# wq2012/SpectralCluster

Measured on AMD Instinct MI355X. Metric: predict() calls/sec, n=8192 d=256 ICASSP2018 (GraphCut, eigengap k in [2,20], cosine k-means), higher is better.
Workload: dtype f64; 1 GPU; icassp2018_graphcut_n8192_d256_k8_max20; n_samples=8192, n_features=256, parallelism=replicas x1, collectives=none

## Files before the change

### spectralcluster_amd/csrc/diffuse_free.hip

```cpp
#include <algorithm>
#include <cstring>
#include <mutex>

#include "dpp.h"
#include "sc_internal.h"

namespace sc {

typedef int v4i __attribute__((ext_vector_type(4)));
typedef int v16i __attribute__((ext_vector_type(16)));

namespace {

__device__ __forceinline__ double fr_wave_max(double v) {
#pragma unroll
  for (int o = 32; o > 0; o >>= 1) v = fmax(v, __shfl_xor(v, o));
  return v;
}
__device__ __forceinline__ double fr_wave_sum(double v) {
#pragma unroll
  for (int o = 32; o > 0; o >>= 1) v += __shfl_xor(v, o);
  return v;
}
__device__ __forceinline__ double fr_block_max(double v, double* sm) {
// ... 574 lines not shown
__global__ __launch_bounds__(kI8Threads) void k_gemm_i8_sym_g(const GroupOf<I8GroupItem> g) {
  const I8GroupItem& a = g.s[blockIdx.y];
  const int nt = (a.n + kI8Tile - 1) / kI8Tile;
  if (a.n <= 0 || (int)blockIdx.x >= nt * (nt + 1) / 2) return;
  const int Kp = (a.n + 63) / 64 * 64;
  I8Split sp{0, 1, nullptr};
  sp.plan = a.plan;
  sp.cus = 0;
  sp.total = a.total;
  gemm_i8_sym_body<0>(a.Q, (size_t)2 * Kp, Kp / 64, a.tilemap, 0, a.T32, nt, a.n, a.M, nullptr, sp);
}

__global__ __launch_bounds__(kI8Threads) void k_i8_tail_finish(
    const int* __restrict__ wsp, int parts, int full_tiles, const int2* __restrict__ tilemap,
    float* __restrict__ T32, int nt, int n, unsigned* __restrict__ M,
    const int* __restrict__ plan, int cus, int nstages, const int* __restrict__ total) {
  const int tt = blockIdx.x, cq = blockIdx.y, cb = cq >> 2, q = cq & 3;
  int I, J;
  if (plan != nullptr) {
    __shared__ int pref[512];
    const int count = *total;
    int r;
    i8_split_plan(count, cus, nstages, &r, &parts);
    if (parts < 2 || tt >= r) return;
    plan_scan(plan, nt, pref);
    __syncthreads();
    full_tiles = count - r;
    plan_lookup(plan, nt, pref, full_tiles + tt, &I, &J);
  } else {
    const int2 tij = tilemap[full_tiles + tt];
    I = tij.x;
    J = tij.y;
  }
  const int lane = threadIdx.x & 63, w = threadIdx.x >> 6;
  const int rr = lane & 31, g = lane >> 5, wr = w >> 1, wc = w & 1;
  const int4* ws = reinterpret_cast<const int4*>(wsp) + (size_t)tt * parts * 24 * kI8Threads + threadIdx.x;
  int4 a = make_int4(0, 0, 0, 0), b = a, c = a;
  for (int p = 0; p < parts; ++p) {
    const int4* src = ws + (size_t)p * 24 * kI8Threads;
    const int4 x = src[(size_t)cq * kI8Threads];
    const int4 y = src[(size_t)(8 + cq) * kI8Threads];
    const int4 z = src[(size_t)(16 + cq) * kI8Threads];
    a.x += x.x; a.y += x.y; a.z += x.z; a.w += x.w;
    b.x += y.x; b.y += y.y; b.z += y.z; b.w += y.w;
    c.x += z.x; c.y += z.y; c.z += z.z; c.w += z.w;
  }
  const int hh[4] = {a.x, a.y, a.z, a.w}, mid[4] = {b.x, b.y, b.z, b.w}, ll[4] = {c.x, c.y, c.z, c.w};
  float* out = T32 + (size_t)tile_to_slot(I, J, nt) * (kI8Tile * kI8Tile);
  const int col = 64 * wc + 32 * cb + rr;
  const bool col_ok = J * kI8Tile + col < n;
  float colm = -INFINITY;
#pragma unroll
  for (int e = 0; e < 4; ++e) {
    const int row = 32 * wr + e + 8 * q + 4 * g;
    const double t = (double)hh[e] * 65536.0 + (double)mid[e] * 256.0 + (double)ll[e];
    const float tf = (float)t;
    out[row * kI8Tile + col] = tf;
    if (I * kI8Tile + row < n) colm = fmaxf(colm, tf);
    float v = col_ok ? tf : -INFINITY;
#pragma unroll
    for (int o = 16; o > 0; o >>= 1) v = fmaxf(v, __shfl_xor(v, o));
    if (rr == 0 && I * kI8Tile + row < n && v > -INFINITY)
      atomicMax(&M[I * kI8Tile + row], ordered_bits(v));
  }
  colm = fmaxf(colm, __shfl_xor(colm, 32));
  if (g == 0 && I != J && J * kI8Tile + col < n && colm > -INFINITY)
    atomicMax(&M[J * kI8Tile + col], ordered_bits(colm));
}

__device__ __forceinline__ void free_append(int row, int col, int cap, int* __restrict__ count,
                                            int* __restrict__ cand) {
  const int pos = atomicAdd(&count[row], 1);
  if (pos < cap) cand[(size_t)row * cap + pos] = col;
}

__device__ __forceinline__ void t32_candidates_body(
    const float* __restrict__ T32, int nt, int n, const unsigned* __restrict__ M,
    const double* __restrict__ R, const unsigned long long* __restrict__ rmax_bits, int cap,
    int* __restrict__ count, int* __restrict__ cand, const int* __restrict__ plan) {
  __shared__ float thrI[128], thrJ[128];
  int I, J;
  size_t slot = blockIdx.x;
  if (plan != nullptr) {
    __shared__ int pref[512];
    const int tiles_run = count[n + kPlanTotalWord];
    if (blockIdx.x == 0 && threadIdx.x == 0) count[n + 67] = tiles_run;
    if ((int)blockIdx.x >= tiles_run) return;
    plan_scan(plan, nt, pref);
    __syncthreads();
    plan_lookup(plan, nt, pref, blockIdx.x, &I, &J);
    slot = tile_to_slot(I, J, nt);
  } else {
    slot_to_tile(blockIdx.x, nt, &I, &J);
    if (blockIdx.x == 0 && threadIdx.x == 0) count[n + 67] = nt * (nt + 1) / 2;
  }
  const float* tile = T32 + slot * (kI8Tile * kI8Tile);
  const int r0 = I * kI8Tile, c0 = J * kI8Tile;
  const int c4 = 4 * (threadIdx.x & 31);
  float4 tv[16];
#pragma unroll
  for (int rg = 0; rg < 16; ++rg)
    tv[rg] = *reinterpret_cast<const float4*>(tile + (8 * rg + (threadIdx.x >> 5)) * kI8Tile + c4);
  const double Rmax = __longlong_as_double((long long)*rmax_bits);
  if (blockIdx.x == 0 && threadIdx.x == 0 && rmax_bits[1] != 0ull) atomicMax(count + n, 1 << 20);
  if (threadIdx.x < 128) {
    const int row = r0 + threadIdx.x;
    thrI[threadIdx.x] = row < n ? free_threshold(ordered_value(M[row]), R[row], Rmax, n) : INFINITY;
  } else {
    const int row = c0 + threadIdx.x - 128;
    thrJ[threadIdx.x - 128] =
        (row < n && I != J) ? free_threshold(ordered_value(M[row]), R[row], Rmax, n) : INFINITY;
  }
  __syncthreads();
  const float tj0 = thrJ[c4], tj1 = thrJ[c4 + 1], tj2 = thrJ[c4 + 2], tj3 = thrJ[c4 + 3];
  const float tjmin = fminf(fminf(tj0, tj1), fminf(tj2, tj3));
#pragma unroll
  for (int rg = 0; rg < 16; ++rg) {
    const int r = 8 * rg + (threadIdx.x >> 5);
    const float4 v = tv[rg];
    const float ti = thrI[r];
    const float vmax = fmaxf(fmaxf(v.x, v.y), fmaxf(v.z, v.w));
    if (vmax >= ti) {
      const int c = c0 + c4;
      if (v.x >= ti && c < n) free_append(r0 + r, c, cap, count, cand);
      if (v.y >= ti && c + 1 < n) free_append(r0 + r, c + 1, cap, count, cand);
      if (v.z >= ti && c + 2 < n) free_append(r0 + r, c + 2, cap, count, cand);
      if (v.w >= ti && c + 3 < n) free_append(r0 + r, c + 3, cap, count, cand);
    }
    if (vmax >= tjmin && r0 + r < n) {
      if (v.x >= tj0) free_append(c0 + c4, r0 + r, cap, count, cand);
      if (v.y >= tj1) free_append(c0 + c4 + 1, r0 + r, cap, count, cand);
      if (v.z >= tj2) free_append(c0 + c4 + 2, r0 + r, cap, count, cand);
      if (v.w >= tj3) free_append(c0 + c4 + 3, r0 + r, cap, count, cand);
    }
  }
}
__global__ __launch_bounds__(256) void k_t32_candidates(
    const float* __restrict__ T32, int nt, int n, const unsigned* __restrict__ M,
    const double* __restrict__ R, const unsigned long long* __restrict__ rmax_bits, int cap,
    int* __restrict__ count, int* __restrict__ cand, const int* __restrict__ plan) {
  t32_candidates_body(T32, nt, n, M, R, rmax_bits, cap, count, cand, plan);
}
__global__ __launch_bounds__(256) void k_t32_candidates_g(const GroupOf<FreeItem> g, int cap) {
  const FreeItem& a = g.s[blockIdx.y];
  const int nt = (a.n + kI8Tile - 1) / kI8Tile;
  if (a.n <= 0 || (int)blockIdx.x >= nt * (nt + 1) / 2) return;
  t32_candidates_body(a.T32, nt, a.n, reinterpret_cast<const unsigned*>(a.words), a.R,
                      reinterpret_cast<const unsigned long long*>(a.scal) + 2, cap, a.words + a.n,
                      a.cand, a.plan);
}


constexpr int kFreeCapMax = 8;
template <int CNT, int U>
__device__ __forceinline__ void free_row_dots(const double* __restrict__ x,
                                               const double* const* __restrict__ xj,
                                               const bool* self, const double* __restrict__ y1,
                                               int n, double* rs_out, double* acc_out) {
  double rs = 0.0;
  double acc[CNT > 0 ? CNT : 1];
#pragma unroll
  for (int c = 0; c < CNT; ++c) acc[c] = 0.0;
  for (int k0 = 2 * threadIdx.x; k0 < n; k0 += 512 * U) {
    double2 a[U], yy[U], b[U][CNT > 0 ? CNT : 1];
#pragma unroll
    for (int u = 0; u < U; ++u) {
      const int k = k0 + 512 * u;
      const bool in = k < n;
      a[u] = in ? *reinterpret_cast<const double2*>(x + k) : make_double2(0.0, 0.0);
      yy[u] = in ? *reinterpret_cast<const double2*>(y1 + k) : make_double2(0.0, 0.0);
#pragma unroll
      for (int c = 0; c < CNT; ++c)
        b[u][c] = (in && !self[c]) ? *reinterpret_cast<const double2*>(xj[c] + k)
                                   : make_double2(0.0, 0.0);
    }
#pragma unroll
    for (int u = 0; u < U; ++u) {
      const int k = k0 + 512 * u;
      if (k + 1 >= n) {
        a[u].y = 0.0;
        yy[u].y = 0.0;
#pragma unroll
        for (int c = 0; c < CNT; ++c) b[u][c].y = 0.0;
      }
      rs = __builtin_fma(a[u].x, yy[u].x, rs);
      rs = __builtin_fma(a[u].y, yy[u].y, rs);
#pragma unroll
      for (int c = 0; c < CNT; ++c) {
        const double2 bb = self[c] ? a[u] : b[u][c];
        acc[c] = __builtin_fma(a[u].x, bb.x, acc[c]);
        acc[c] = __builtin_fma(a[u].y, bb.y, acc[c]);
      }
    }
  }
  *rs_out = rs;
#pragma unroll
  for (int c = 0; c < CNT; ++c) acc_out[c] = acc[c];
}

__device__ __forceinline__ void free_row_stats_body(
    const double* __restrict__ A, int n, int ld, const double* __restrict__ y1,
    const int* __restrict__ count, const int* __restrict__ cand, int cap,
    double* __restrict__ rowmax, double* __restrict__ rowsum, int* __restrict__ ovf) {
  __shared__ double sm[4];
  const int row = blockIdx.x;
  const int total = count[row];
  const int cnt = total < cap ? total : cap;
  const double* x = A + (size_t)row * ld;
  const double* xj[kFreeCapMax];
  bool self[kFreeCapMax];
#pragma unroll
  for (int c = 0; c < kFreeCapMax; ++c) {
    const int j = c < cnt ? cand[(size_t)row * cap + c] : row;
    self[c] = j == row;
    xj[c] = A + (size_t)j * ld;
  }
  double acc[kFreeCapMax];
#pragma unroll
  for (int c = 0; c < kFreeCapMax; ++c) acc[c] = 0.0;
  double rs = 0.0;
  switch (cnt) {
    case 0: free_row_dots<0, 4>(x, xj, self, y1, n, &rs, acc); break;
    case 1: free_row_dots<1, 4>(x, xj, self, y1, n, &rs, acc); break;
    case 2: free_row_dots<2, 4>(x, xj, self, y1, n, &rs, acc); break;
    case 3: free_row_dots<3, 2>(x, xj, self, y1, n, &rs, acc); break;
    case 4: free_row_dots<4, 2>(x, xj, self, y1, n, &rs, acc); break;
    default: free_row_dots<kFreeCapMax, 1>(x, xj, self, y1, n, &rs, acc); break;
  }
  rs = fr_block_sum(rs, sm);
  double best = -INFINITY;
#pragma unroll
  for (int c = 0; c < kFreeCapMax; ++c) {
    if (c < cnt) {
      const double d = fr_block_sum(acc[c], sm);
      best = fmax(best, d);
    }
  }
  if (threadIdx.x == 0) {
    rowmax[row] = best;
    rowsum[row] = rs;
    if (total > cap) {
      const int e = atomicAdd(&ovf[0], 1);
      if (e < 64) ovf[1 + e] = row;
    }
  }
  if (row == 0) {
    int sum = 0, big = 0;
    for (int i = threadIdx.x; i < n; i += 256) {
      const int t = count[i];
      sum += t < cap ? t : cap;
      big = t > big ? t : big;
    }
#pragma unroll
    for (int o = 32; o > 0; o >>= 1) {
      sum += __shfl_xor(sum, o);
      const int other = __shfl_xor(big, o);
      big = other > big ? other : big;
    }
    __shared__ int ssum[4], sbig[4];
    if ((threadIdx.x & 63) == 0) {
      ssum[threadIdx.x >> 6] = sum;
      sbig[threadIdx.x >> 6] = big;
    }
    __syncthreads();
    if (threadIdx.x == 0) {
      ovf[65] = (ssum[0] + ssum[1]) + (ssum[2] + ssum[3]);
      ovf[66] = max(max(sbig[0], sbig[1]), max(sbig[2], sbig[3]));
    }
  }
}
__global__ __launch_bounds__(256) void k_free_row_stats(
    const double* __restrict__ A, int n, int ld, const double* __restrict__ y1,
    const int* __restrict__ count, const int* __restrict__ cand, int cap,
    double* __restrict__ rowmax, double* __restrict__ rowsum, int* __restrict__ ovf) {
  free_row_stats_body(A, n, ld, y1, count, cand, cap, rowmax, rowsum, ovf);
}
__global__ __launch_bounds__(256) void k_free_row_stats_g(const GroupOf<FreeItem> g, int cap) {
  const FreeItem& a = g.s[blockIdx.y];
  if ((int)blockIdx.x >= a.n) return;
  free_row_stats_body(a.A, a.n, a.ld, a.y1, a.words + a.n, a.cand, cap, a.rowmax, a.rowsum,
                       a.words + 2 * (size_t)a.n);
}

__global__ __launch_bounds__(256) void k_free_gather_rows(const double* __restrict__ A, int n,
                                                          int ld, const int* __restrict__ rows,
                                                          int nrows, double* __restrict__ Vs) {
  const int v = threadIdx.x & (kEigBlock - 1);
  const int k = blockIdx.x * (256 / kEigBlock) + threadIdx.x / kEigBlock;
  if (k >= n) return;
  Vs[(size_t)k * kEigBlock + v] = v < nrows ? A[(size_t)rows[v] * ld + k] : 0.0;
}
__global__ __launch_bounds__(256) void k_free_colmax(const double* __restrict__ W, int n,
                                                     const int* __restrict__ rows, int nrows,
                                                     double* __restrict__ rowmax) {
  __shared__ double sm[4];
  const int v = blockIdx.x;
  if (v >= nrows) return;
  double m = -INFINITY;
  for (int k = threadIdx.x; k < n; k += 256) m = fmax(m, W[(size_t)k * kEigBlock + v]);
  m = fr_block_max(m, sm);
  if (threadIdx.x == 0) rowmax[rows[v]] = m;
}

int free_rows_padded(int n) { return round_up(n, kI8Tile); }
int free_k_padded(int n) { return round_up(n, 64); }
size_t free_q_bytes(int n) { return (size_t)free_rows_padded(n) * 2 * free_k_padded(n); }
size_t free_t32_bytes(int n) {
  const size_t nt = (n + kI8Tile - 1) / kI8Tile;
  return nt * (nt + 1) / 2 * kI8Tile * kI8Tile * sizeof(float);
}
int free_candidate_cap() { return kFreeCapMax; }

void launch_free_absmax(hipStream_t s, const double* A, int n, int ld, double* scal) {
  hipLaunchKernelGGL(k_free_absmax, dim3(n), dim3(256), 0, s, A, n, ld,
                     reinterpret_cast<unsigned long long*>(scal));
}

void launch_free_amax_from_cut(hipStream_t s, const double* cut, int n, double p,
                               double floor_value, double* scal) {
  hipLaunchKernelGGL(k_free_amax_from_cut, dim3(1), dim3(256), 0, s, cut, n, p, floor_value, scal);
}

void launch_free_quantize(hipStream_t s, const double* A, int n, int ld, signed char* Q,
                          double* scal, double* y1, double* R, double* q2part) {
  const int Kp = free_k_padded(n);
  SC_OPT_IN_LDS(k_free_quantize<0>, 2 * 65536);
  hipLaunchKernelGGL(k_free_quantize<0>, dim3(free_rows_padded(n)), dim3(256), (size_t)2 * Kp, s, A,
                     n, ld, Q, (size_t)2 * Kp, Kp, scal, y1, R,
                     reinterpret_cast<unsigned long long*>(scal) + 2, q2part);
}
size_t free_q2part_bytes(int n) { return (size_t)free_k_padded(n) * (free_k_padded(n) / 64) * sizeof(double); }
size_t free_mx64_bytes(int n) { return (size_t)(free_k_padded(n) / 64) * (free_k_padded(n) / 64) * sizeof(double); }
size_t free_tau64_bytes(int n) { return (size_t)(free_k_padded(n) / 64) * sizeof(float); }
size_t free_plan_bytes(int n) {
  const size_t nt = (n + kI8Tile - 1) / kI8Tile;
  return (nt + nt * nt) * sizeof(int);
}
void launch_free_seg_reduce(hipStream_t s, const double* R, int n, const FreeSegs& segs) {
  const int nblk = free_k_padded(n) / 64;
  hipLaunchKernelGGL(k_free_seg_reduce, dim3(nblk), dim3(256), 0, s, R, n, nblk, segs);
}
void launch_free_tile_flags(hipStream_t s, const double* mx64, const float* tau64, int n,
                            int* plan, bool prune, int* words) {
  const int nt = (n + kI8Tile - 1) / kI8Tile;
  hipLaunchKernelGGL(k_free_tile_flags, dim3(nt), dim3(kFlagThreads), 0, s, mx64, tau64, nt,
                     free_k_padded(n) / 64, plan, prune ? 1 : 0,
                     words + 2 * (size_t)n + kPlanTotalWord);
}

static int device_cus() {
  static int cus = 0;
  if (cus == 0) {
    int dev = 0, v = 0;
    if (hipGetDevice(&dev) == hipSuccess &&
        hipDeviceGetAttribute(&v, hipDeviceAttributeMultiprocessorCount, dev) == hipSuccess && v > 0)
      cus = v;
    else
      cus = 256;
  }
  return cus;
}
void free_i8_split_plan(int n, int* tail_tiles, int* parts) {
  const int nt = (n + kI8Tile - 1) / kI8Tile;
  const int tiles = nt * (nt + 1) / 2;
  const int stages = free_k_padded(n) / 64;
  const int cus = device_cus();
  *tail_tiles = 0;
  *parts = 1;
  const int r = tiles % cus;
  if (tiles <= cus || r == 0 || 2 * r > cus) return;
  for (int f = std::min(8, cus / r); f >= 2; --f)
    if (stages % f == 0 && stages / f >= 4) {
      *tail_tiles = r;
      *parts = f;
      return;
    }
}
size_t free_i8_split_bytes(int n) {
  int r, f;
  free_i8_split_plan(n, &r, &f);
  return f > 1 ? (size_t)r * f * 96 * kI8Threads * sizeof(int) : 0;
}
size_t free_i8_split_bytes_plan() { return (size_t)device_cus() * 96 * kI8Threads * sizeof(int); }

void launch_gemm_i8_sym(hipStream_t s, const signed char* Q, int n, const int2* tilemap,
                        float* T32, unsigned* M, int* split_ws, const int* plan) {
  const int nt = (n + kI8Tile - 1) / kI8Tile;
  const int tiles = nt * (nt + 1) / 2;
  const int Kp = free_k_padded(n);
  const int lds = kI8Buffers * kI8StageBytes;
  if (plan != nullptr && split_ws != nullptr) {
    const int cus = device_cus();
    I8Split sp{0, 1, split_ws};
    sp.plan = plan;
    sp.cus = cus;
    sp.total = reinterpret_cast<const int*>(M) + 2 * (size_t)n + kPlanTotalWord;
    SC_OPT_IN_LDS(k_gemm_i8_sym<0>, lds);
    hipLaunchKernelGGL(k_gemm_i8_sym<0>, dim3(tiles + cus), dim3(kI8Threads), lds, s, Q,
                       (size_t)2 * Kp, Kp / 64, tilemap, 0, T32, nt, n, M,
                       static_cast<unsigned long long*>(nullptr), sp);
    hipLaunchKernelGGL(k_i8_tail_finish, dim3(cus / 2, 8), dim3(kI8Threads), 0, s, split_ws, 1, 0,
                       tilemap, T32, nt, n, M, plan, cus, Kp / 64, sp.total);
    return;
  }
  int r = 0, f = 1;
  if (split_ws != nullptr) free_i8_split_plan(n, &r, &f);
  const int full = tiles - r;
  const int xcd_chunk = (full % 8 == 0 && full >= 512) ? full / 8 : 0;
  SC_OPT_IN_LDS(k_gemm_i8_sym<0>, lds);
  hipLaunchKernelGGL(k_gemm_i8_sym<0>, dim3(full + r * f), dim3(kI8Threads), lds, s, Q,
                     (size_t)2 * Kp, Kp / 64, tilemap, xcd_chunk, T32, nt, n, M,
                     static_cast<unsigned long long*>(nullptr), I8Split{full, f, split_ws});
  if (f > 1)
    hipLaunchKernelGGL(k_i8_tail_finish, dim3(r, 8), dim3(kI8Threads), 0, s, split_ws, f, full,
                       tilemap, T32, nt, n, M, static_cast<const int*>(nullptr), 0, 0,
                       static_cast<const int*>(nullptr));
}

void launch_gemm_i8_sym_group(hipStream_t s, const signed char* const* Q, float* const* T32,
                              unsigned* const* M, int count, const int* ns,
                              const int2* const* tilemaps, const int* const* plans) {
  const int lds = kI8Buffers * kI8StageBytes;
  SC_OPT_IN_LDS(k_gemm_i8_sym_g, lds);
  GroupOf<I8GroupItem> g;
  memset(&g, 0, sizeof(g));
  int tiles = 0;
  for (int z = 0; z < count; ++z) {
    g.s[z] = I8GroupItem{Q[z], T32[z], M[z], tilemaps[z], ns[z], plans ? plans[z] : nullptr,
                         reinterpret_cast<const int*>(M[z]) + 2 * (size_t)ns[z] + kPlanTotalWord};
    const int nt = (ns[z] + kI8Tile - 1) / kI8Tile;
    tiles = std::max(tiles, nt * (nt + 1) / 2);
  }
  if (tiles == 0) return;
  hipLaunchKernelGGL(k_gemm_i8_sym_g, dim3(tiles, count), dim3(kI8Threads), lds, s, g);
}

void launch_t32_candidates(hipStream_t s, const float* T32, int n, const unsigned* M,
                           const double* R, const double* scal, int* count, int* cand,
                           const int* plan) {
  const int nt = (n + kI8Tile - 1) / kI8Tile;
  hipLaunchKernelGGL(k_t32_candidates, dim3(nt * (nt + 1) / 2), dim3(256), 0, s, T32, nt, n, M, R,
                     reinterpret_cast<const unsigned long long*>(scal) + 2, kFreeCapMax, count,
                     cand, plan);
}

void launch_free_row_stats(hipStream_t s, const double* A, int n, int ld, const double* y1,
                           const int* count, const int* cand, double* rowmax, double* rowsum,
                           int* ovf) {
  hipLaunchKernelGGL(k_free_row_stats, dim3(n), dim3(256), 0, s, A, n, ld, y1, count, cand,
                     kFreeCapMax, rowmax, rowsum, ovf);
}

static GroupOf<FreeItem> free_pack(const FreeItem* items, int count, int* nmax) {
  GroupOf<FreeItem> g;
  memset(&g, 0, sizeof(g));
  *nmax = 0;
  for (int z = 0; z < count; ++z) {
    g.s[z] = items[z];
    *nmax = std::max(*nmax, items[z].n);
  }
  return g;
}
void launch_free_begin_group(hipStream_t s, const FreeItem* items, int count, double floor_value,
                             bool pad_rows) {
  int nmax;
  const GroupOf<FreeItem> g = free_pack(items, count, &nmax);
  if (nmax == 0) return;
  const int nwords = 2 * nmax + kFreeOvfWords;
  hipLaunchKernelGGL(k_free_begin_g, dim3(1 + (nwords + 1023) / 1024 + (pad_rows ? 32 : 0), count),
                     dim3(256), 0, s, g, floor_value, pad_rows ? 1 : 0);
}
void launch_free_tile_flags_group(hipStream_t s, const FreeItem* items, int count, bool prune) {
  int nmax;
  const GroupOf<FreeItem> g = free_pack(items, count, &nmax);
  if (nmax == 0) return;
  hipLaunchKernelGGL(k_free_tile_flags_g, dim3((nmax + kI8Tile - 1) / kI8Tile, count),
                     dim3(kFlagThreads), 0, s, g, prune ? 1 : 0);
}
void launch_free_scan_stats_group(hipStream_t s, const FreeItem* items, int count) {
  int nmax;
  const GroupOf<FreeItem> g = free_pack(items, count, &nmax);
  if (nmax == 0) return;
  const int nt = (nmax + kI8Tile - 1) / kI8Tile;
  hipLaunchKernelGGL(k_t32_candidates_g, dim3(nt * (nt + 1) / 2, count), dim3(256), 0, s, g,
                     kFreeCapMax);
  hipLaunchKernelGGL(k_free_row_stats_g, dim3(nmax, count), dim3(256), 0, s, g, kFreeCapMax);
}

void launch_free_gather_rows(hipStream_t s, const double* A, int n, int ld, const int* rows,
                             int nrows, double* Vs) {
  const int per = 256 / kEigBlock;
  hipLaunchKernelGGL(k_free_gather_rows, dim3((n + per - 1) / per), dim3(256), 0, s, A, n, ld,
                     rows, nrows, Vs);
}

void launch_free_colmax(hipStream_t s, const double* W, int n, const int* rows, int nrows,
                        double* rowmax) {
  hipLaunchKernelGGL(k_free_colmax, dim3(nrows), dim3(256), 0, s, W, n, rows, nrows, rowmax);
}

}
```

### spectralcluster_amd/csrc/eig.hip

```cpp
#include <algorithm>
#include <cstring>
#include <mutex>

#include "sc_internal.h"

namespace sc {

typedef double v4f64 __attribute__((ext_vector_type(4)));
constexpr int B = kEigBlock;
constexpr int RB = 256 / B;
static_assert(B == 8 || B == 16, "block width must divide the 16-wide MFMA tile");

__device__ __forceinline__ uint64_t splitmix64(uint64_t x) {
  x += 0x9E3779B97F4A7C15ull;
  x = (x ^ (x >> 30)) * 0xBF58476D1CE4E5B9ull;
  x = (x ^ (x >> 27)) * 0x94D049BB133111EBull;
  return x ^ (x >> 31);
}
__device__ __forceinline__ double hash_uniform(uint64_t seed, uint64_t idx) {
  const uint64_t h = splitmix64(seed ^ splitmix64(idx));
  return (double)(h >> 11) * (2.0 / 9007199254740992.0) - 1.0;
}

__global__ void k_random_block(double* W, int n, uint64_t seed) {
// ... 68 lines not shown
      if (row < n && li < B)
        W[(size_t)row * B + li] =
            __builtin_fma(cvec ? cvec[row] : 1.0, sum,
                          pvec ? pvec[row] * V[(size_t)row * ldv + li] : 0.0);
    }
  }
}
__global__ __launch_bounds__(64 * kMvWaves) void k_block_matvec(
    const double* __restrict__ S, int ld, int n, const double* __restrict__ cvec,
    const double* __restrict__ pvec, const double* __restrict__ V, int ldv,
    const double* __restrict__ Vs, double* __restrict__ W) {
  block_matvec_body(S, ld, n, cvec, pvec, V, ldv, Vs, W);
}
__global__ __launch_bounds__(64 * kMvWaves) void k_block_matvec_g(const GroupOf<MatvecItem> g) {
  const MatvecItem& a = g.s[blockIdx.y];
  if ((int)blockIdx.x * 16 >= a.n) return;
  block_matvec_body(a.S, a.ld, a.n, a.cvec, a.pvec, a.V, a.ldv, a.Vs, a.W);
}

constexpr int kSymTile = 128;
constexpr int kSymPitch = 34;
__device__ __forceinline__ int sym_item_id(int I, int J, int nt) {
  return I * nt - I * (I - 1) / 2 + (J - I);
}
__device__ __forceinline__ void block_matvec_sym_body(
    const double* __restrict__ S, int ld, int n, const double* __restrict__ Vs,
    double* __restrict__ pdirect, double* __restrict__ pmirror, int nt) {
  __shared__ __attribute__((aligned(16))) double smem[4 * 32 * kSymPitch];
  int I = 0, rem = blockIdx.x, rowlen = nt;
  while (rem >= rowlen) {
    rem -= rowlen;
    --rowlen;
    ++I;
  }
  const int J = I + rem;
  const bool diag = I == J;
  const int lane = threadIdx.x & 63, wave = threadIdx.x >> 6;
  const int li = lane & 15, lg = lane >> 4;
  const int r0 = I * kSymTile + 32 * wave;
  const int c0 = J * kSymTile;
  double* patch = smem + wave * (32 * kSymPitch);
  double bm[8];
#pragma unroll
  for (int t = 0; t < 8; ++t) {
    const int row = r0 + 4 * t + lg;
    bm[t] = (row < n && li < B) ? Vs[(size_t)row * B + li] : 0.0;
  }
  v4f64 accd[2] = {{0.0, 0.0, 0.0, 0.0}, {0.0, 0.0, 0.0, 0.0}};
  v4f64 accm[4][2];
#pragma unroll
  for (int cs = 0; cs < 4; ++cs)
#pragma unroll
    for (int ct = 0; ct < 2; ++ct) accm[cs][ct] = (v4f64){0.0, 0.0, 0.0, 0.0};
  double2 a[1][2][4];
  auto load = [&](int buf, int cs) {
#pragma unroll
    for (int rt = 0; rt < 2; ++rt) {
      int row = r0 + 16 * rt + li;
      row = row < n ? row : n - 1;
      const double* src = S + (size_t)row * ld + c0 + 32 * cs + 2 * lg;
#pragma unroll
      for (int q = 0; q < 4; ++q) {
        if (c0 + 32 * cs + 8 * q + 2 * lg + 1 < ld)
          a[buf][rt][q] = *reinterpret_cast<const double2*>(src + 8 * q);
        else
          a[buf][rt][q] = make_double2(0.0, 0.0);
      }
    }
  };
#pragma unroll
  for (int cs = 0; cs < 4; ++cs) {
    constexpr int cur = 0;
    load(cur, cs);
    const int kb = c0 + 32 * cs + 2 * lg;
#pragma unroll
    for (int rt = 0; rt < 2; ++rt) {
      const bool rok = r0 + 16 * rt + li < n;
#pragma unroll
      for (int q = 0; q < 4; ++q) {
        if (!rok || kb + 8 * q >= n) a[cur][rt][q].x = 0.0;
        if (!rok || kb + 8 * q + 1 >= n) a[cur][rt][q].y = 0.0;
      }
    }
    double b[8];
#pragma unroll
    for (int t = 0; t < 8; ++t) {
      const int k = kb + 8 * (t >> 1) + (t & 1);
      b[t] = (k < n && li < B) ? Vs[(size_t)k * B + li] : 0.0;
    }
#pragma unroll
    for (int rt = 0; rt < 2; ++rt)
#pragma unroll
      for (int q = 0; q < 4; ++q) {
        accd[rt] = __builtin_amdgcn_mfma_f64_16x16x4f64(a[cur][rt][q].x, b[2 * q], accd[rt], 0, 0, 0);
        accd[rt] = __builtin_amdgcn_mfma_f64_16x16x4f64(a[cur][rt][q].y, b[2 * q + 1], accd[rt], 0, 0, 0);
      }
    if (!diag) {
#pragma unroll
      for (int rt = 0; rt < 2; ++rt)
#pragma unroll
        for (int q = 0; q < 4; ++q)
          *reinterpret_cast<double2*>(patch + (16 * rt + li) * kSymPitch + 8 * q + 2 * lg) =
              a[cur][rt][q];
      __builtin_amdgcn_fence(__ATOMIC_RELEASE, "wavefront");
      __builtin_amdgcn_wave_barrier();
#pragma unroll
      for (int ct = 0; ct < 2; ++ct)
#pragma unroll
        for (int t = 0; t < 8; ++t) {
          const double at = patch[(4 * t + lg) * kSymPitch + 16 * ct + li];
          accm[cs][ct] = __builtin_amdgcn_mfma_f64_16x16x4f64(at, bm[t], accm[cs][ct], 0, 0, 0);
        }
      __builtin_amdgcn_fence(__ATOMIC_ACQUIRE, "wavefront");
      __builtin_amdgcn_wave_barrier();
    }
  }
  const size_t item = blockIdx.x;
  if (li < B) {
#pragma unroll
    for (int rt = 0; rt < 2; ++rt)
#pragma unroll
      for (int r = 0; r < 4; ++r)
        pdirect[(item * kSymTile + 32 * wave + 16 * rt + lg + 4 * r) * B + li] = accd[rt][r];
  }
  if (diag) return;
  __syncthreads();
  double* red = smem;
  if (li < B) {
#pragma unroll
    for (int cs = 0; cs < 4; ++cs)
#pragma unroll
      for (int ct = 0; ct < 2; ++ct)
#pragma unroll
        for (int r = 0; r < 4; ++r)
          red[(wave * kSymTile + 32 * cs + 16 * ct + lg + 4 * r) * B + li] = accm[cs][ct][r];
  }
  __syncthreads();
  for (int e = threadIdx.x; e < kSymTile * B; e += 256)
    pmirror[item * (kSymTile * B) + e] =
        ((red[e] + red[kSymTile * B + e]) + red[2 * kSymTile * B + e]) + red[3 * kSymTile * B + e];
}
__global__ __launch_bounds__(256) void k_block_matvec_sym(
    const double* __restrict__ S, int ld, int n, const double* __restrict__ Vs,
    double* __restrict__ pdirect, double* __restrict__ pmirror, int nt) {
  block_matvec_sym_body(S, ld, n, Vs, pdirect, pmirror, nt);
}
__global__ __launch_bounds__(256) void k_block_matvec_sym_g(const GroupOf<MatvecItem> g) {
  const MatvecItem& a = g.s[blockIdx.y];
  const int nt = (a.n + kSymTile - 1) / kSymTile;
  if ((int)blockIdx.x >= nt * (nt + 1) / 2) return;
  block_matvec_sym_body(a.S, a.ld, a.n, a.Vs, a.slabs, a.slabs + (size_t)(nt * (nt + 1) / 2) * kSymTile * B, nt);
}

__device__ __forceinline__ void matvec_sym_reduce_body(
    const double* __restrict__ pdirect, const double* __restrict__ pmirror, int nt, int n,
    const double* __restrict__ cvec, const double* __restrict__ pvec,
    const double* __restrict__ V, int ldv, double* __restrict__ W) {
  const int R = blockIdx.x / 4;
  const int e = (blockIdx.x & 3) * 256 + threadIdx.x;
  const int rl = e / B, v = e % B;
  const int row = R * kSymTile + rl;
  double acc = 0.0;
  const int total = nt;
  for (int s0 = 0; s0 < total; s0 += 8) {
    double x[8];
#pragma unroll
    for (int u = 0; u < 8; ++u) {
      const int sidx = s0 + u;
      x[u] = 0.0;
      if (sidx < nt - R) {
        x[u] = pdirect[(size_t)sym_item_id(R, R + sidx, nt) * (kSymTile * B) + e];
      } else if (sidx < total) {
        x[u] = pmirror[(size_t)sym_item_id(sidx - (nt - R), R, nt) * (kSymTile * B) + e];
      }
    }
#pragma unroll
    for (int u = 0; u < 8; ++u) acc += x[u];
  }
  if (row < n) W[(size_t)row * B + v] =
      __builtin_fma(cvec ? cvec[row] : 1.0, acc, pvec ? pvec[row] * V[(size_t)row * ldv + v] : 0.0);
}
__global__ __launch_bounds__(256) void k_matvec_sym_reduce(
    const double* __restrict__ pdirect, const double* __restrict__ pmirror, int nt, int n,
    const double* __restrict__ cvec, const double* __restrict__ pvec,
    const double* __restrict__ V, int ldv, double* __restrict__ W) {
  matvec_sym_reduce_body(pdirect, pmirror, nt, n, cvec, pvec, V, ldv, W);
}
__global__ __launch_bounds__(256) void k_matvec_sym_reduce_g(const GroupOf<MatvecItem> g) {
  const MatvecItem& a = g.s[blockIdx.y];
  const int nt = (a.n + kSymTile - 1) / kSymTile;
  if ((int)blockIdx.x >= nt * 4) return;
  matvec_sym_reduce_body(a.slabs, a.slabs + (size_t)(nt * (nt + 1) / 2) * kSymTile * B, nt, a.n,
                         a.cvec, a.pvec, a.V, a.ldv, a.W);
}

constexpr int kProjGroups = 256 / B;
constexpr int kProjAcc = (kLdq + kProjGroups - 1) / kProjGroups;
__global__ __launch_bounds__(256) void k_proj_partial(
    const double* __restrict__ Q, int ldq, int m, const double* __restrict__ W,
    int n, double* __restrict__ partial) {
  __shared__ double Ql[8][kLdq];
  __shared__ double Wl[8][B];
  const int tid = threadIdx.x;
  const int jj = tid % B, ig = tid / B;
  const int rows_per = (n + gridDim.x - 1) / gridDim.x;
  const int rbeg = blockIdx.x * rows_per;
  const int rend = min(n, rbeg + rows_per);
  double acc[kProjAcc];
#pragma unroll
  for (int q = 0; q < kProjAcc; ++q) acc[q] = 0.0;
  for (int r = rbeg; r < rend; r += 8) {
    __syncthreads();
    for (int e = tid; e < 8 * m; e += 256) {
      const int rr = e / m, i = e - rr * m;
      Ql[rr][i] = (r + rr < rend) ? Q[(size_t)(r + rr) * ldq + i] : 0.0;
    }
    if (tid < 8 * B) {
      const int rr = tid / B;
      Wl[rr][jj] = (r + rr < rend) ? W[(size_t)(r + rr) * B + jj] : 0.0;
    }
    __syncthreads();
#pragma unroll
    for (int rr = 0; rr < 8; ++rr) {
      const double w = Wl[rr][jj];
#pragma unroll
      for (int q = 0; q < kProjAcc; ++q)
        if (ig + kProjGroups * q < m)
          acc[q] = __builtin_fma(Ql[rr][ig + kProjGroups * q], w, acc[q]);
    }
  }
  double* out = partial + (size_t)blockIdx.x * (kLdq * B);
#pragma unroll
  for (int q = 0; q < kProjAcc; ++q)
    if (ig + kProjGroups * q < m) out[(ig + kProjGroups * q) * B + jj] = acc[q];
}

__global__ __launch_bounds__(256) void k_reduce_H(
    const double* __restrict__ partial, int nparts, int m, double* __restrict__ Hbuf,
    double* __restrict__ T, int ldt, int col0, int accumulate,
    double* __restrict__ hsq) {
  __shared__ double sq[32];
  const int tid = threadIdx.x;
  const int sub = tid & 7;
  const int e = blockIdx.x * 32 + (tid >> 3);
  double h = 0.0;
  if (e < m * B)
    for (int g = sub; g < nparts; g += 8) h += partial[(size_t)g * (kLdq * B) + e];
  h += __shfl_xor(h, 1);
  h += __shfl_xor(h, 2);
  h += __shfl_xor(h, 4);
  if (sub == 0) {
    if (e < m * B) {
      Hbuf[e] = h;
      if (T != nullptr) {
        const int i = e / B, j = col0 + (e % B);
        if (i <= j) {
          const double v = accumulate ? T[(size_t)i * ldt + j] + h : h;
          T[(size_t)i * ldt + j] = v;
          T[(size_t)j * ldt + i] = v;
        }
      }
    } else {
      h = 0.0;
    }
    sq[tid >> 3] = h * h;
  }
  __syncthreads();
  if (tid < B) {
    double s = 0.0;
    for (int q = tid; q < 32; q += B) s += sq[q];
    atomicAdd(&hsq[tid], s);
  }
}

__global__ __launch_bounds__(256) void k_update_block(
    const double* __restrict__ Q, int ldq, int m, const double* __restrict__ Hbuf,
    double* __restrict__ W, int n) {
  __shared__ double Hl[kLdq * B];
  __shared__ double Ql[RB][kLdq + 1];
  const int tid = threadIdx.x;
  const int jj = tid % B, rr = tid / B;
  const int r0 = blockIdx.x * RB;
  for (int e = tid; e < m * B; e += 256) Hl[e] = Hbuf[e];
  for (int e = tid; e < RB * m; e += 256) {
    const int a = e / m, i = e - a * m;
    Ql[a][i] = (r0 + a < n) ? Q[(size_t)(r0 + a) * ldq + i] : 0.0;
  }
  __syncthreads();
  const int r = r0 + rr;
  if (r < n) {
    double acc = W[(size_t)r * B + jj];
    for (int i = 0; i < m; ++i) acc = __builtin_fma(-Ql[rr][i], Hl[i * B + jj], acc);
    W[(size_t)r * B + jj] = acc;
  }
}

__device__ __forceinline__ void chol8_wave(const double* G, double* __restrict__ Rinv,
                                           const double* __restrict__ hsq,
                                           int* __restrict__ flags,
                                           int* __restrict__ defect_flag, int flag_mode,
                                           int* __restrict__ sticky_flag = nullptr,
                                           int sticky_m = 0, bool sticky_on_defect = true);

__global__ __launch_bounds__(256) void k_reduce_chol(
    const double* __restrict__ partial, int nparts, double* __restrict__ Rinv,
    double* __restrict__ Gsave, const double* __restrict__ hsq,
    int* __restrict__ flags, int* __restrict__ defect_flag, int flag_mode) {
  static_assert(B == 8, "the factorisation below maps the 8 x 8 matrix onto one wavefront");
  __shared__ double G[B * B];
  const int tid = threadIdx.x;
  {
    constexpr int kLanes = 256 / (B * B);
    const int e = tid / kLanes, sub = tid % kLanes;
    double g = 0.0;
    for (int q = sub; q < nparts; q += kLanes) g += partial[(size_t)q * (kLdq * B) + e];
#pragma unroll
    for (int o = 1; o < kLanes; o <<= 1) g += __shfl_xor(g, o);
    if (sub == 0) {
      G[e] = g;
      if (Gsave) Gsave[e] = g;
    }
  }
  __syncthreads();
  if (tid >= 64) return;
  chol8_wave(G, Rinv, hsq, flags, defect_flag, flag_mode);
}

__device__ __forceinline__ void chol8_wave(const double* G, double* __restrict__ Rinv,
                                           const double* __restrict__ hsq,
                                           int* __restrict__ flags,
// ... 965 lines not shown
```

Measured before the change: 385.9 calls/s.

## Process two rows per block in free row stats and widen sym-reduce batch

The free-row-stats kernel now handles two rows per block. When a candidate neighbour is the other row in the block, its data comes from the already-loaded row registers instead of a second global read, and the block reductions are merged into a single shared-memory pass with one barrier. The launch grids are halved to match. Separately, the symmetric matvec reduction loads 32 partial slabs per batch instead of 8 to expose more memory-level parallelism. The cost is higher register pressure and more template instantiations.

```diff
diff --git a/spectralcluster_amd/csrc/diffuse_free.hip b/spectralcluster_amd/csrc/diffuse_free.hip
--- a/spectralcluster_amd/csrc/diffuse_free.hip
+++ b/spectralcluster_amd/csrc/diffuse_free.hip
@@ -750,99 +750,159 @@
 
 
 constexpr int kFreeCapMax = 8;
-template <int CNT, int U>
-__device__ __forceinline__ void free_row_dots(const double* __restrict__ x,
-                                               const double* const* __restrict__ xj,
-                                               const bool* self, const double* __restrict__ y1,
-                                               int n, double* rs_out, double* acc_out) {
-  double rs = 0.0;
-  double acc[CNT > 0 ? CNT : 1];
-#pragma unroll
-  for (int c = 0; c < CNT; ++c) acc[c] = 0.0;
+constexpr int kFreeRows = 2;
+template <int RR, int CNT, int U>
+__device__ __forceinline__ void free_rows_dots(const double* __restrict__ A, int ld, int first,
+                                                const int (*jj)[kFreeCapMax],
+                                                const double* __restrict__ y1, int n,
+                                                double* rs_out, double (*acc_out)[kFreeCapMax]) {
+  constexpr int C1 = CNT > 0 ? CNT : 1;
+  const double* x[RR];
+  const double* xj[RR][C1];
+  int reg[RR][C1];
+#pragma unroll
+  for (int r = 0; r < RR; ++r) {
+    const int row = first + r < n ? first + r : n - 1;
+    x[r] = A + (size_t)row * ld;
+#pragma unroll
+    for (int c = 0; c < CNT; ++c) {
+      const int j = jj[r][c];
+      const int g = j < 0 ? r : j - first;
+      reg[r][c] = (g >= 0 && g < RR) ? g : -1;
+      xj[r][c] = A + (size_t)(j < 0 ? row : j) * ld;
+    }
+  }
+  double rs[RR], acc[RR][C1];
+#pragma unroll
+  for (int r = 0; r < RR; ++r) {
+    rs[r] = 0.0;
+#pragma unroll
+    for (int c = 0; c < CNT; ++c) acc[r][c] = 0.0;
+  }
   for (int k0 = 2 * threadIdx.x; k0 < n; k0 += 512 * U) {
-    double2 a[U], yy[U], b[U][CNT > 0 ? CNT : 1];
+    double2 a[U][RR], yy[U], b[U][RR][C1];
 #pragma unroll
     for (int u = 0; u < U; ++u) {
       const int k = k0 + 512 * u;
       const bool in = k < n;
-      a[u] = in ? *reinterpret_cast<const double2*>(x + k) : make_double2(0.0, 0.0);
       yy[u] = in ? *reinterpret_cast<const double2*>(y1 + k) : make_double2(0.0, 0.0);
 #pragma unroll
-      for (int c = 0; c < CNT; ++c)
-        b[u][c] = (in && !self[c]) ? *reinterpret_cast<const double2*>(xj[c] + k)
-                                   : make_double2(0.0, 0.0);
+      for (int r = 0; r < RR; ++r) {
+        a[u][r] = in ? *reinterpret_cast<const double2*>(x[r] + k) : make_double2(0.0, 0.0);
+#pragma unroll
+        for (int c = 0; c < CNT; ++c)
+          b[u][r][c] = (in && reg[r][c] < 0) ? *reinterpret_cast<const double2*>(xj[r][c] + k)
+                                             : make_double2(0.0, 0.0);
+      }
     }
 #pragma unroll
     for (int u = 0; u < U; ++u) {
       const int k = k0 + 512 * u;
       if (k + 1 >= n) {
-        a[u].y = 0.0;
         yy[u].y = 0.0;
 #pragma unroll
-        for (int c = 0; c < CNT; ++c) b[u][c].y = 0.0;
+        for (int r = 0; r < RR; ++r) {
+          a[u][r].y = 0.0;
+#pragma unroll
+          for (int c = 0; c < CNT; ++c) b[u][r][c].y = 0.0;
+        }
       }
-      rs = __builtin_fma(a[u].x, yy[u].x, rs);
-      rs = __builtin_fma(a[u].y, yy[u].y, rs);
-#pragma unroll
-      for (int c = 0; c < CNT; ++c) {
-        const double2 bb = self[c] ? a[u] : b[u][c];
-        acc[c] = __builtin_fma(a[u].x, bb.x, acc[c]);
-        acc[c] = __builtin_fma(a[u].y, bb.y, acc[c]);
+#pragma unroll
+      for (int r = 0; r < RR; ++r) {
+        rs[r] = __builtin_fma(a[u][r].x, yy[u].x, rs[r]);
+        rs[r] = __builtin_fma(a[u][r].y, yy[u].y, rs[r]);
+#pragma unroll
+        for (int c = 0; c < CNT; ++c) {
+          double2 bb = b[u][r][c];
+#pragma unroll
+          for (int g = 0; g < RR; ++g)
+            if (reg[r][c] == g) bb = a[u][g];
+          acc[r][c] = __builtin_fma(a[u][r].x, bb.x, acc[r][c]);
+          acc[r][c] = __builtin_fma(a[u][r].y, bb.y, acc[r][c]);
+        }
       }
     }
   }
-  *rs_out = rs;
-#pragma unroll
-  for (int c = 0; c < CNT; ++c) acc_out[c] = acc[c];
+#pragma unroll
+  for (int r = 0; r < RR; ++r) {
+    rs_out[r] = rs[r];
+#pragma unroll
+    for (int c = 0; c < CNT; ++c) acc_out[r][c] = acc[r][c];
+  }
+}
+template <int RR, int CNT, int U>
+__device__ __forceinline__ void free_rows_split(const double* __restrict__ A, int ld, int row0,
+                                                 const int (*jj)[kFreeCapMax],
+                                                 const double* __restrict__ y1, int n, double* rs,
+                                                 double (*acc)[kFreeCapMax]) {
+#pragma unroll
+  for (int r = 0; r < kFreeRows; r += RR)
+    if (row0 + r < n) free_rows_dots<RR, CNT, U>(A, ld, row0 + r, jj + r, y1, n, rs + r, acc + r);
 }
 
 __device__ __forceinline__ void free_row_stats_body(
     const double* __restrict__ A, int n, int ld, const double* __restrict__ y1,
     const int* __restrict__ count, const int* __restrict__ cand, int cap,
     double* __restrict__ rowmax, double* __restrict__ rowsum, int* __restrict__ ovf) {
-  __shared__ double sm[4];
-  const int row = blockIdx.x;
-  const int total = count[row];
-  const int cnt = total < cap ? total : cap;
-  const double* x = A + (size_t)row * ld;
-  const double* xj[kFreeCapMax];
-  bool self[kFreeCapMax];
-#pragma unroll
-  for (int c = 0; c < kFreeCapMax; ++c) {
-    const int j = c < cnt ? cand[(size_t)row * cap + c] : row;
-    self[c] = j == row;
-    xj[c] = A + (size_t)j * ld;
-  }
-  double acc[kFreeCapMax];
-#pragma unroll
-  for (int c = 0; c < kFreeCapMax; ++c) acc[c] = 0.0;
-  double rs = 0.0;
-  switch (cnt) {
-    case 0: free_row_dots<0, 4>(x, xj, self, y1, n, &rs, acc); break;
-    case 1: free_row_dots<1, 4>(x, xj, self, y1, n, &rs, acc); break;
-    case 2: free_row_dots<2, 4>(x, xj, self, y1, n, &rs, acc); break;
-    case 3: free_row_dots<3, 2>(x, xj, self, y1, n, &rs, acc); break;
-    case 4: free_row_dots<4, 2>(x, xj, self, y1, n, &rs, acc); break;
-    default: free_row_dots<kFreeCapMax, 1>(x, xj, self, y1, n, &rs, acc); break;
-  }
-  rs = fr_block_sum(rs, sm);
-  double best = -INFINITY;
-#pragma unroll
-  for (int c = 0; c < kFreeCapMax; ++c) {
-    if (c < cnt) {
-      const double d = fr_block_sum(acc[c], sm);
-      best = fmax(best, d);
-    }
-  }
-  if (threadIdx.x == 0) {
+  static_assert(kFreeRows == 2 || kFreeRows == 4, "the step counts below are chosen for 2 and 4");
+  constexpr int R = kFreeRows;
+  __shared__ double sm[R][1 + kFreeCapMax][4];
+  const int row0 = blockIdx.x * R;
+  int cnt[R], jj[R][kFreeCapMax];
+  int cmax = 0;
+#pragma unroll
+  for (int r = 0; r < R; ++r) {
+    const int row = row0 + r;
+    const int total = row < n ? count[row] : 0;
+    cnt[r] = total < cap ? total : cap;
+    cmax = cnt[r] > cmax ? cnt[r] : cmax;
+#pragma unroll
+    for (int c = 0; c < kFreeCapMax; ++c) jj[r][c] = c < cnt[r] ? cand[(size_t)row * cap + c] : -1;
+  }
+  double rs[R], acc[R][kFreeCapMax];
+#pragma unroll
+  for (int r = 0; r < R; ++r) {
+    rs[r] = 0.0;
+#pragma unroll
+    for (int c = 0; c < kFreeCapMax; ++c) acc[r][c] = 0.0;
+  }
+  switch (cmax) {
+    case 0: free_rows_split<R, 0, 8 / R>(A, ld, row0, jj, y1, n, rs, acc); break;
+    case 1: free_rows_split<R, 1, 8 / R>(A, ld, row0, jj, y1, n, rs, acc); break;
+    case 2: free_rows_split<R, 2, 4 / R>(A, ld, row0, jj, y1, n, rs, acc); break;
+    case 3: free_rows_split<2, 3, 1>(A, ld, row0, jj, y1, n, rs, acc); break;
+    case 4: free_rows_split<2, 4, 1>(A, ld, row0, jj, y1, n, rs, acc); break;
+    default: free_rows_split<1, kFreeCapMax, 1>(A, ld, row0, jj, y1, n, rs, acc); break;
+  }
+  const int lane = threadIdx.x & 63, wave = threadIdx.x >> 6;
+#pragma unroll
+  for (int r = 0; r < R; ++r) {
+    const double v = fr_wave_sum(rs[r]);
+    if (lane == 0) sm[r][0][wave] = v;
+#pragma unroll
+    for (int c = 0; c < kFreeCapMax; ++c) {
+      if (c < cnt[r]) {
+        const double d = fr_wave_sum(acc[r][c]);
+        if (lane == 0) sm[r][1 + c][wave] = d;
+      }
+    }
+  }
+  __syncthreads();
+  if (threadIdx.x < R && row0 + (int)threadIdx.x < n) {
+    const int r = threadIdx.x, row = row0 + r;
+    const int total = count[row];
+    const int mine = total < cap ? total : cap;
+    double best = -INFINITY;
+    for (int c = 0; c < mine; ++c)
+      best = fmax(best, (sm[r][1 + c][0] + sm[r][1 + c][1]) + (sm[r][1 + c][2] + sm[r][1 + c][3]));
     rowmax[row] = best;
-    rowsum[row] = rs;
+    rowsum[row] = (sm[r][0][0] + sm[r][0][1]) + (sm[r][0][2] + sm[r][0][3]);
     if (total > cap) {
       const int e = atomicAdd(&ovf[0], 1);
       if (e < 64) ovf[1 + e] = row;
     }
   }
-  if (row == 0) {
+  if (blockIdx.x == 0) {
     int sum = 0, big = 0;
     for (int i = threadIdx.x; i < n; i += 256) {
       const int t = count[i];
@@ -875,7 +935,7 @@
 }
 __global__ __launch_bounds__(256) void k_free_row_stats_g(const GroupOf<FreeItem> g, int cap) {
   const FreeItem& a = g.s[blockIdx.y];
-  if ((int)blockIdx.x >= a.n) return;
+  if ((int)blockIdx.x * kFreeRows >= a.n) return;
   free_row_stats_body(a.A, a.n, a.ld, a.y1, a.words + a.n, a.cand, cap, a.rowmax, a.rowsum,
                        a.words + 2 * (size_t)a.n);
 }
@@ -1045,7 +1105,7 @@
 void launch_free_row_stats(hipStream_t s, const double* A, int n, int ld, const double* y1,
                            const int* count, const int* cand, double* rowmax, double* rowsum,
                            int* ovf) {
-  hipLaunchKernelGGL(k_free_row_stats, dim3(n), dim3(256), 0, s, A, n, ld, y1, count, cand,
+  hipLaunchKernelGGL(k_free_row_stats, dim3((n + kFreeRows - 1) / kFreeRows), dim3(256), 0, s, A, n, ld, y1, count, cand,
                      kFreeCapMax, rowmax, rowsum, ovf);
 }
 
@@ -1082,7 +1142,8 @@
   const int nt = (nmax + kI8Tile - 1) / kI8Tile;
   hipLaunchKernelGGL(k_t32_candidates_g, dim3(nt * (nt + 1) / 2, count), dim3(256), 0, s, g,
                      kFreeCapMax);
-  hipLaunchKernelGGL(k_free_row_stats_g, dim3(nmax, count), dim3(256), 0, s, g, kFreeCapMax);
+  hipLaunchKernelGGL(k_free_row_stats_g, dim3((nmax + kFreeRows - 1) / kFreeRows, count),
+                     dim3(256), 0, s, g, kFreeCapMax);
 }
 
 void launch_free_gather_rows(hipStream_t s, const double* A, int n, int ld, const int* rows,
diff --git a/spectralcluster_amd/csrc/eig.hip b/spectralcluster_amd/csrc/eig.hip
--- a/spectralcluster_amd/csrc/eig.hip
+++ b/spectralcluster_amd/csrc/eig.hip
@@ -244,6 +244,7 @@
   block_matvec_sym_body(a.S, a.ld, a.n, a.Vs, a.slabs, a.slabs + (size_t)(nt * (nt + 1) / 2) * kSymTile * B, nt);
 }
 
+constexpr int kSymReduceBatch = 32;
 __device__ __forceinline__ void matvec_sym_reduce_body(
     const double* __restrict__ pdirect, const double* __restrict__ pmirror, int nt, int n,
     const double* __restrict__ cvec, const double* __restrict__ pvec,
@@ -254,10 +255,10 @@
   const int row = R * kSymTile + rl;
   double acc = 0.0;
   const int total = nt;
-  for (int s0 = 0; s0 < total; s0 += 8) {
-    double x[8];
-#pragma unroll
-    for (int u = 0; u < 8; ++u) {
+  for (int s0 = 0; s0 < total; s0 += kSymReduceBatch) {
+    double x[kSymReduceBatch];
+#pragma unroll
+    for (int u = 0; u < kSymReduceBatch; ++u) {
       const int sidx = s0 + u;
       x[u] = 0.0;
       if (sidx < nt - R) {
@@ -267,7 +268,7 @@
       }
     }
 #pragma unroll
-    for (int u = 0; u < 8; ++u) acc += x[u];
+    for (int u = 0; u < kSymReduceBatch; ++u) acc += x[u];
   }
   if (row < n) W[(size_t)row * B + v] =
       __builtin_fma(cvec ? cvec[row] : 1.0, acc, pvec ? pvec[row] * V[(size_t)row * ldv + v] : 0.0);
```

Result: no change. 383.7 calls/s (-0.6%).
